# Arcadia-Science/arcadia-microscopy-tools

Measured on AMD Instinct MI355X. Metric: fields-of-view/sec (4x2048^2 uint16) end-to-end segment+props, higher is better.
Workload: dtype f64; 1 GPU; configs[2]: synthetic 4-channel 2048x2048 uint16 FOVs, DAPI Gaussian+Otsu+open/close+EDT+peak markers+watershed nuclei (SEEDED relief, seeds_first: marker pixels spread first in raster order, cannot tie; SURVEY A.8's plain -EDT relief with exact ties is reported under sublines.a8_exact) + clear_border/relabel + morphology and 4-channel intensity regionprops; mode=weak scaling, 192 FOVs per GPU per step, streams_per_gpu=4, fovs_per_launch=48, max_cells_per_fov=2048, distinct_fovs_per_gpu=8, resident_in_hbm=True

## Files before the change

### arcadia_microscopy_tools_amd/csrc/amt_props.hip

```cpp
#include "amt_internal.h"
#include "amt_perlabel.h"

#include <vector>

typedef unsigned long long u64;

enum { A_N = 0, A_SY, A_SX, A_SYY, A_SXX, A_SXY, A_C1, A_C2, A_C3, A_NACC };

__global__ void __launch_bounds__(256) rp_init_kernel(u64* __restrict__ acc, int* __restrict__ bbox, size_t nlab) {
    for (size_t i = (size_t)blockIdx.x * 256 + threadIdx.x; i < nlab; i += (size_t)gridDim.x * 256) {
        if (acc)
            for (int k = 0; k < A_NACC; ++k) acc[i * A_NACC + k] = 0;
        bbox[i * 4 + 0] = 0x7fffffff;
        bbox[i * 4 + 1] = 0x7fffffff;
        bbox[i * 4 + 2] = -1;
        bbox[i * 4 + 3] = -1;
    }
}

__device__ __forceinline__ double diff_of_products(u64 a, u64 b, u64 c, u64 d) {
    u64 lo1 = a * b, hi1 = __umul64hi(a, b);
    u64 lo2 = c * d, hi2 = __umul64hi(c, d);
    bool neg = (hi1 < hi2) || (hi1 == hi2 && lo1 < lo2);
    u64 hi, lo;
    if (!neg) {
        lo = lo1 - lo2;
        hi = hi1 - hi2 - (lo1 < lo2 ? 1 : 0);
    } else {
        lo = lo2 - lo1;
        hi = hi2 - hi1 - (lo2 < lo1 ? 1 : 0);
    }
    double v = (double)hi * 18446744073709551616.0 + (double)lo;
    return neg ? -v : v;
}

__global__ void __launch_bounds__(256) rp_bbox_kernel(const int* __restrict__ labels, int* __restrict__ bbox, int H,
                                                      int W, int max_label) {
    const int lane = threadIdx.x & 63;
    const int x = blockIdx.x * 64 + lane;
    const int yb = (blockIdx.y * 4 + (threadIdx.x >> 6)) * 8;
    if (yb >= H) return;
    const size_t n = (size_t)H * W;
    const int plane = blockIdx.z;
    int labs[8];
#pragma unroll
    for (int k = 0; k < 8; ++k) {
        const int y = yb + k;
        int v = 0;
        if (x < W && y < H) v = labels[(size_t)plane * n + (size_t)y * W + x];
        labs[k] = (v < 0 || v > max_label) ? 0 : v;
    }
#pragma unroll
    for (int k = 0; k < 8; ++k) {
        const int lab = labs[k];
        const int left = __shfl_up(lab, 1);
        const bool head = (lane == 0) || (left != lab);
        const u64 heads = __ballot(head);
        if (lab != 0 && head) {
            const u64 later = heads & ~((2ull << lane) - 1ull);
            const int end_lane = later ? (__ffsll((long long)later) - 2) : 63;
            int* B = bbox + ((size_t)plane * max_label + (lab - 1)) * 4;
            atomicMin(&B[0], yb + k);
            atomicMin(&B[1], x);
            atomicMax(&B[2], yb + k);
            atomicMax(&B[3], x + (end_lane - lane));
        }
    }
}

int amt_i_label_boxes(amt_ctx* ctx, const int* labels, int* bbox, unsigned long long* acc, int nplanes, int H, int W,
                      int max_label) {
    const size_t nlab = (size_t)nplanes * max_label;
    hipLaunchKernelGGL(rp_init_kernel, dim3(amt_grid_for(nlab, 256, 1024)), dim3(256), 0, ctx->stream, acc, bbox, nlab);
    AMT_LAUNCH_CHECK();
    hipLaunchKernelGGL(rp_bbox_kernel, dim3((W + 63) / 64, (H + 31) / 32, nplanes), dim3(256), 0, ctx->stream, labels, bbox,
                       H, W, max_label);
    AMT_LAUNCH_CHECK();
    return AMT_OK;
}

constexpr int RP_MAXC = 4;
constexpr int RPS = 3;
__device__ __forceinline__ size_t rp_uniform(size_t v) {
    const unsigned lo = (unsigned)__builtin_amdgcn_readfirstlane((int)(unsigned)v);
    const unsigned hi = (unsigned)__builtin_amdgcn_readfirstlane((int)(unsigned)(v >> 32));
    return ((size_t)hi << 32) | lo;
}
struct RpSums {
    u64 cnt, sy, sx, syy, sxx, sxy;
    u64 s[RP_MAXC], q[RP_MAXC];
    unsigned mn[RP_MAXC], mx[RP_MAXC];
};

template <int LC>
__device__ __forceinline__ void rp_label_scan(const int* __restrict__ L, const uint16_t* __restrict__ I, size_t n, int W,
                                              int x0, int y0, int x1, int y1, int want, int nc, bool rows_ok,
                                              int2* __restrict__ myrows, int lane, RpSums& a) {
    constexpr int COLS = 1 << LC, RW = 64 >> LC;
    const int col = lane & (COLS - 1), sub = lane >> LC;
    size_t cofs[RP_MAXC];
#pragma unroll
    for (int c = 0; c < RP_MAXC; ++c) cofs[c] = rp_uniform((size_t)(c < nc ? c : 0) * n);
    int lv[RPS];
    unsigned iv[RPS][RP_MAXC] = {};
    auto load_step = [&](int yb, int xb) {
        const int xr = x1 - xb;
        const unsigned cx = (unsigned)(col <= xr ? col : xr);
#pragma unroll
        for (int j = 0; j < RPS; ++j) {
            const int yt = yb + j * RW, ys = yt <= y1 ? yt : y1;
            const int y = yt + sub, yc = y <= y1 ? y : y1;
            const unsigned off = (unsigned)(yc - ys) * (unsigned)W + cx;
            const size_t base = (size_t)ys * W + xb;
            lv[j] = *(const int*)((const char*)(L + base) + off * 4u);
            if (I) {
#pragma unroll
                for (int c = 0; c < RP_MAXC; ++c)
                    iv[j][c] = *(const uint16_t*)((const char*)(I + cofs[c] + base) + off * 2u);
            }
        }
    };
    int nyb = y0, nxb = x0;
    int rmin[RPS], rmax[RPS];
    unsigned tcnt = 0;
    u64 tsy = 0;
    do {
        const int yb = nyb, xb = nxb;
        load_step(yb, xb);
        nxb = xb + 64;
        if (LC < 6 || nxb > x1) {
            nxb = x0;
            nyb = yb + RPS * RW;
        }
        const int x = xb + col;
        if (LC == 6 && xb == x0) {
#pragma unroll
            for (int j = 0; j < RPS; ++j) {
                rmin[j] = 0x7fffffff;
                rmax[j] = -1;
            }
        }
        unsigned bcnt = 0, bsy = 0;
        int2* steprows = myrows + (yb - y0 + sub);
#pragma unroll
        for (int j = 0; j < RPS; ++j) {
            const int y = yb + j * RW + sub;
            const bool m = x <= x1 && y <= y1 && lv[j] == want;
            if (m) {
                bcnt += 1u;
                bsy += (unsigned)y;
                a.syy += (u64)(unsigned)y * (unsigned)y;
                if (I) {
#pragma unroll
                    for (int c = 0; c < RP_MAXC; ++c) {
                        const unsigned v = iv[j][c];
                        a.s[c] += v;
                        a.q[c] += (u64)v * v;
                        a.mn[c] = v < a.mn[c] ? v : a.mn[c];
                        a.mx[c] = v > a.mx[c] ? v : a.mx[c];
                    }
                }
            }
            const u64 bal = __ballot(m);
            if constexpr (LC == 6) {
                if (bal) {
                    const int first = xb + __ffsll((long long)bal) - 1;
                    const int last = xb + 63 - __clzll((long long)bal);
                    rmin[j] = first < rmin[j] ? first : rmin[j];
                    rmax[j] = last > rmax[j] ? last : rmax[j];
                }
            } else {
                const unsigned sm = (unsigned)(bal >> (sub * COLS)) & (0xffffffffu >> (32 - COLS));
                if (rows_ok && col == 0 && y <= y1)
                    steprows[j * RW] = sm ? make_int2(x0 + __ffs((int)sm) - 1, x0 + 31 - __clz((int)sm))
                                          : make_int2(0x7fffffff, -1);
            }
        }
        if constexpr (LC == 6) {
            a.cnt += bcnt;
            a.sy += bsy;
            a.sx += (u64)(unsigned)x * bcnt;
            a.sxx += (u64)(unsigned)x * (unsigned)x * bcnt;
            a.sxy += (u64)(unsigned)x * bsy;
            if (rows_ok && lane == 0 && nxb == x0) {
#pragma unroll
                for (int j = 0; j < RPS; ++j)
                    if (yb + j <= y1) myrows[yb + j - y0] = make_int2(rmin[j], rmax[j]);
            }
        } else {
            tcnt += bcnt;
            tsy += bsy;
        }
    } while (nyb <= y1);
    if constexpr (LC < 6) {
        const unsigned x = (unsigned)(x0 + col);
        a.cnt = tcnt;
        a.sy = tsy;
        a.sx = (u64)x * tcnt;
        a.sxx = (u64)x * x * tcnt;
        a.sxy = (u64)x * tsy;
    }
}

__global__ void __launch_bounds__(64) rp_label_kernel(const int* __restrict__ labels, const int* __restrict__ bbox,
                                                      const int* __restrict__ hoff, const int* __restrict__ htot,
                                                      int2* __restrict__ rows, size_t cap, u64* __restrict__ acc,
                                                      const uint16_t* __restrict__ inten, int C, int c0, int nc,
                                                      double* __restrict__ itable, int H, int W, int max_label,
                                                      int want_morph) {
    const int plane = blockIdx.y;
    const int l = blockIdx.x;
    const int lane = threadIdx.x;
    const size_t li = (size_t)plane * max_label + l;
    const amt_box box = amt_load_box(bbox, li);
    const int y0 = box.y0, x0 = box.x0, y1 = box.y1, x1 = box.x1;
    if (box.absent()) {
        if (itable) amt_fill_row(itable + (li * C + c0) * 4, 4 * nc, 0.0, lane);
        return;
    }
    const size_t n = (size_t)H * W;
    const int* L = labels + (size_t)plane * n;
    const uint16_t* I = inten ? inten + ((size_t)plane * C + c0) * n : nullptr;
    const bool rows_ok = want_morph && (size_t)htot[plane] <= cap;
    int2* myrows = rows + (size_t)plane * cap + (size_t)hoff[li];
    RpSums a;
    a.cnt = a.sy = a.sx = a.syy = a.sxx = a.sxy = 0;
#pragma unroll
    for (int c = 0; c < RP_MAXC; ++c) {
        a.s[c] = 0;
        a.q[c] = 0;
        a.mn[c] = 0xffffffffu;
        a.mx[c] = 0;
    }
    const int w = W < (1 << 28) ? x1 - x0 + 1 : 64;
    if (w <= 16) rp_label_scan<4>(L, I, n, W, x0, y0, x1, y1, l + 1, nc, rows_ok, myrows, lane, a);
    else if (w <= 32) rp_label_scan<5>(L, I, n, W, x0, y0, x1, y1, l + 1, nc, rows_ok, myrows, lane, a);
    else rp_label_scan<6>(L, I, n, W, x0, y0, x1, y1, l + 1, nc, rows_ok, myrows, lane, a);
    static_assert(A_N == 0 && A_SXY == 5, "the moment sums are the first six accumulator slots");
    u64 t[16];
    t[A_N] = a.cnt, t[A_SY] = a.sy, t[A_SX] = a.sx, t[A_SYY] = a.syy, t[A_SXX] = a.sxx, t[A_SXY] = a.sxy;
    unsigned e[2 * RP_MAXC];
#pragma unroll
    for (int c = 0; c < RP_MAXC; ++c) {
        t[6 + c] = a.s[c];
        t[6 + RP_MAXC + c] = a.q[c];
        e[c] = a.mn[c];
        e[RP_MAXC + c] = ~a.mx[c];
    }
    t[14] = t[15] = 0;
    const u64 red = amt_wave_reduce_scatter<16, amt_op_sum>(t, lane);
    if (want_morph && (lane & 3) == 0 && lane < 4 * 6) acc[li * A_NACC + (lane >> 2)] = red;
    if (itable) {
        const unsigned ext = amt_wave_reduce_scatter<8, amt_op_min>(e, lane);
        const u64 cnt = __shfl(red, 0), S = __shfl(red, 4 * (6 + lane)), Q = __shfl(red, 4 * (6 + RP_MAXC + lane));
        const unsigned lo = __shfl(ext, 8 * lane), hi = ~__shfl(ext, 8 * (RP_MAXC + lane));
        if (lane < nc) {
            double* o = itable + (li * C + c0 + lane) * 4;
            if (cnt == 0) {
                o[0] = o[1] = o[2] = o[3] = 0.0;
            } else {
                const double dn = (double)cnt;
                o[0] = (double)S / dn;
                o[1] = (double)hi;
                o[2] = (double)lo;
                const double nv = diff_of_products(cnt, Q, S, S);
                const double var = nv / (dn * dn);
                o[3] = sqrt(var < 0.0 ? 0.0 : var);
            }
        }
    }
}

constexpr int PR_ROWS = 64, PR_IN = 60, PR_BATCH = 17, PR_NBATCH = (PR_ROWS + 4) / PR_BATCH;
static_assert(PR_BATCH * PR_NBATCH == PR_ROWS + 4, "row batches must tile the strip");

__global__ void __launch_bounds__(256) rp_perimeter_rows_kernel(const int* __restrict__ labels, u64* __restrict__ acc,
                                                                int H, int W, int max_label, int* __restrict__ bbox) {
    const int lane = threadIdx.x & 63;
    const int strip = blockIdx.x * 4 + (threadIdx.x >> 6);
    if (strip * PR_IN >= W) return;
    const int plane = blockIdx.z;
    const size_t n = (size_t)H * W;
    const int* L = labels + (size_t)plane * n;
    const int x = strip * PR_IN - 2 + lane;
    const int y0 = blockIdx.y * PR_ROWS;
    const bool xin = x >= 0 && x < W;
    const bool inner = xin && lane >= 2 && lane < 2 + PR_IN;
    const unsigned ml = (unsigned)max_label;
    u64* accp = acc + (size_t)plane * max_label * A_NACC;
    int* bbp = bbox ? bbox + (size_t)plane * max_label * 4 : nullptr;

    const int xc = x < 0 ? 0 : (x < W ? x : W - 1);
    auto load_row = [&](int y) -> int {
        const int yc = y < 0 ? 0 : (y < H ? y : H - 1);
        return L[(size_t)yc * W + xc];
    };
    int cur[PR_BATCH], nxt[PR_BATCH];
#pragma unroll
    for (int j = 0; j < PR_BATCH; ++j) cur[j] = load_row(y0 - 2 + j);
    int v1 = 0, v1l = 0, v1r = 0, v2 = 0, v2l = 0, v2r = 0;
    int wA = 0, wAl = 0, wAr = 0, wB = 0, wBl = 0, wBr = 0;
    for (int b = 0; b < PR_NBATCH; ++b) {
        if (b + 1 < PR_NBATCH) {
#pragma unroll
            for (int j = 0; j < PR_BATCH; ++j) nxt[j] = load_row(y0 - 2 + (b + 1) * PR_BATCH + j);
        }
#pragma unroll
        for (int j = 0; j < PR_BATCH; ++j) {
            const int r = y0 - 2 + b * PR_BATCH + j;
            int v0 = cur[j];
            v0 = (xin && r >= 0 && r < H && (unsigned)(v0 - 1) < ml) ? v0 : 0;
            if (__ballot((v0 | v1 | v2 | wB) != 0) == 0ull) continue;
            const int v0l = amt_lane_left(v0), v0r = amt_lane_right(v0);
            const bool b1 = v1 != 0 && (v2 != v1 || v0 != v1 || v1l != v1 || v1r != v1);
            const int w1 = b1 ? (v1 | (int)0x80000000) : v1;
            const int w1l = amt_lane_left(w1), w1r = amt_lane_right(w1);
            const int yb = r - 1;
            if (bbp && yb >= y0 && yb < y0 + PR_ROWS) {
                const bool live = inner && v1 != 0, head = live && v1l != v1;
                const bool q0 = head && v2 != v1, q2 = head && v0 != v1, q1 = head && v2l != v1 && v0l != v1;
                const bool q3 = live && v1r != v1 && v2r != v1 && v0r != v1;
                if (__ballot(q0 || q1 || q2 || q3)) {
                    int* B = bbp + (size_t)(v1 - 1) * 4;
                    if (q0) atomicMin(&B[0], yb);
                    if (q2) atomicMax(&B[2], yb);
                    if (q1) atomicMin(&B[1], x);
                    if (q3) atomicMax(&B[3], x);
                }
            }
            const int yo = r - 2;
            if (inner && wA < 0 && yo >= y0 && yo < y0 + PR_ROWS) {
                const int key = wA;
                const int code = 1 + 2 * ((wB == key) + (w1 == key) + (wAl == key) + (wAr == key)) +
                                 10 * ((wBl == key) + (wBr == key) + (w1l == key) + (w1r == key));
                constexpr unsigned long long M1 = (1ull << 5) | (1ull << 7) | (1ull << 15) | (1ull << 17) | (1ull << 25) | (1ull << 27);
                constexpr unsigned long long M2 = (1ull << 21) | (1ull << 33), M3 = (1ull << 13) | (1ull << 23);
                const int cls = ((M1 >> code) & 1ull) ? A_C1 : ((M2 >> code) & 1ull) ? A_C2 : ((M3 >> code) & 1ull) ? A_C3 : -1;
                if (cls >= 0) atomicAdd(&accp[(size_t)((key & 0x7fffffff) - 1) * A_NACC + cls], 1ull);
            }
            wB = wA, wBl = wAl, wBr = wAr;
            wA = w1, wAl = w1l, wAr = w1r;
            v2 = v1, v2l = v1l, v2r = v1r;
            v1 = v0, v1l = v0l, v1r = v0r;
        }
#pragma unroll
        for (int j = 0; j < PR_BATCH; ++j) cur[j] = nxt[j];
    }
}

__global__ void __launch_bounds__(256) rp_heights_kernel(const int* __restrict__ bbox, int* __restrict__ hoff,
                                                         int max_label) {
    const int plane = blockIdx.y;
    for (int l = blockIdx.x * 256 + threadIdx.x; l < max_label; l += gridDim.x * 256) {
        const int* B = bbox + ((size_t)plane * max_label + l) * 4;
        hoff[(size_t)plane * max_label + l] = B[2] >= B[0] ? B[2] - B[0] + 1 : 0;
    }
}

constexpr int HULL_HMAX = 48, HULL_WMAX = 250;

__device__ __forceinline__ void rp_write_convex(double* __restrict__ trow, double convex) {
    const double area = trow[AMT_RP_AREA];
    trow[AMT_RP_AREA_CONVEX] = convex;
    trow[AMT_RP_SOLIDITY] = area > 0.0 ? area / convex : 0.0;
}

__device__ __forceinline__ long long floor_div(long long a, long long b) {
    long long q = a / b;
    return (a % b != 0 && a < 0) ? q - 1 : q;
}
__device__ __forceinline__ long long ceil_div(long long a, long long b) {
    long long q = a / b;
    return (a % b != 0 && a > 0) ? q + 1 : q;
}

template <bool CROWS>
__global__ void __launch_bounds__(64) rp_hull_kernel(const int* __restrict__ bbox, const int* __restrict__ hoff,
                                                     const int* __restrict__ htot, const int2* __restrict__ rows,
                                                     int2* __restrict__ chainL, int2* __restrict__ chainR, size_t cap,
                                                     double* __restrict__ table, int max_label, int skip_h,
                                                     int2* __restrict__ crows) {
    const int plane = blockIdx.y;
    const int l = blockIdx.x * 64 + threadIdx.x;
    if (l >= max_label) return;
    const size_t li = (size_t)plane * max_label + l;
    double* trow = CROWS ? nullptr : table + li * AMT_RP_NCOLS;
    const int miny = bbox[li * 4 + 0], maxy = bbox[li * 4 + 2];
    if (maxy < miny) {
        if (!CROWS && skip_h == 0) trow[AMT_RP_AREA_CONVEX] = 0.0;
        return;
    }
    const int h = maxy - miny + 1;
    if (h <= skip_h && bbox[li * 4 + 3] - bbox[li * 4 + 1] + 1 <= HULL_WMAX) return;
    const size_t off = (size_t)hoff[li];
    if ((size_t)htot[plane] > cap || off + (size_t)h > cap) {
        if (!CROWS) rp_write_convex(trow, __longlong_as_double(0x7ff8000000000000ll));
        return;
    }
    const int2* r = rows + (size_t)plane * cap + off;
// ... 209 lines not shown
        const double SQ2 = 1.4142135623730951;
        t[AMT_RP_PERIMETER] = (double)A[A_C1] + (double)A[A_C2] * SQ2 + (double)A[A_C3] * ((1.0 + SQ2) / 2.0);
        const double Nyy = diff_of_products(n, A[A_SYY], A[A_SY], A[A_SY]);
        const double Nxx = diff_of_products(n, A[A_SXX], A[A_SX], A[A_SX]);
        const double Nxy = diff_of_products(n, A[A_SXY], A[A_SX], A[A_SY]);
        const double n2 = dn * dn;
        const double a = Nxx / n2;
        const double c = Nyy / n2;
        const double b = -Nxy / n2;
        const double tr = (a + c) * 0.5;
        const double hd = (a - c) * 0.5;
        const double rad = sqrt(hd * hd + b * b);
        double l1 = tr + rad, l2 = tr - rad;
        l1 = l1 < 0.0 ? 0.0 : l1;
        l2 = l2 < 0.0 ? 0.0 : l2;
        t[AMT_RP_AXIS_MAJOR] = 4.0 * sqrt(l1);
        t[AMT_RP_AXIS_MINOR] = 4.0 * sqrt(l2);
        t[AMT_RP_ECCENTRICITY] = l1 == 0.0 ? 0.0 : sqrt(1.0 - l2 / l1);
        double orient;
        if (Nxx == Nyy) {
            orient = (Nxy > 0.0) ? -0.78539816339744828 : 0.78539816339744828;
        } else {
            orient = 0.5 * atan2(-2.0 * b, c - a);
        }
        t[AMT_RP_ORIENTATION] = orient;
    }
}

extern "C" int amt_regionprops(amt_ctx* ctx, const int32_t* labels, const uint16_t* intensity, int C, double* table_dev,
                               double* itable_dev, int nplanes, int H, int W, int max_label) {
    AMT_REQUIRE(labels && (table_dev || itable_dev) && nplanes >= 0 && H > 0 && W > 0 && max_label >= 0,
                "regionprops: bad arguments");
    AMT_REQUIRE(!intensity == !itable_dev && (!itable_dev || C >= 1),
                "regionprops: the intensity planes (C >= 1) and the intensity table go together");
    AMT_CHECK_OPERANDS("amt_regionprops", amt_in("labels", labels, amt_span(4, nplanes, H, W)),
                       amt_in("intensity", intensity, amt_span(2, nplanes, C, H, W)),
                       amt_out("table_dev", table_dev, amt_span(8, nplanes, max_label, AMT_RP_NCOLS)),
                       amt_out("itable_dev", itable_dev, amt_span(8, nplanes, max_label, C, 4)));
    AMT_TRY(amt_set_device(ctx));
    const bool want_morph = table_dev != nullptr;
    if (nplanes == 0 || max_label == 0) return AMT_OK;
    const size_t n = (size_t)H * W;
    const size_t nlab = (size_t)nplanes * max_label;
    const size_t cap = want_morph ? n : 1;
    amt_scratch s(ctx);
    amt_buf<u64> acc(s, nlab * A_NACC);
    amt_buf<int> bbox(s, nlab * 4);
    amt_buf<int> hoff(s, nlab);
    amt_buf<int> htot(s, nplanes);
    amt_buf<int2> rows(s, (size_t)nplanes * cap);
    amt_buf<int2> chainL(s, (size_t)nplanes * 3 * cap);
    amt_buf<int2> chainR(s, (size_t)nplanes * 3 * cap);
    AMT_TRY(s.commit());
    if (want_morph) {
        hipLaunchKernelGGL(rp_init_kernel, dim3(amt_grid_for(nlab, 256, 1024)), dim3(256), 0, ctx->stream, acc, bbox, nlab);
        AMT_LAUNCH_CHECK();
        const int nstrips = (W + PR_IN - 1) / PR_IN;
        dim3 gper((nstrips + 3) / 4, (H + PR_ROWS - 1) / PR_ROWS, nplanes);
        hipLaunchKernelGGL(rp_perimeter_rows_kernel, gper, dim3(256), 0, ctx->stream, labels, acc, H, W, max_label, bbox);
        AMT_LAUNCH_CHECK();
    } else {
        AMT_TRY(amt_i_label_boxes(ctx, labels, bbox, acc, nplanes, H, W, max_label));
    }
    hipLaunchKernelGGL(rp_heights_kernel, dim3(amt_grid_for(max_label, 256, 256), nplanes), dim3(256), 0, ctx->stream,
                       bbox, hoff, max_label);
    AMT_LAUNCH_CHECK();
    AMT_TRY(amt_scan_excl(ctx, hoff, max_label, (size_t)max_label, htot, nplanes));
    const int groups = intensity ? (C + RP_MAXC - 1) / RP_MAXC : 1;
    for (int g = 0; g < groups; ++g) {
        const int c0 = g * RP_MAXC;
        const int nc = intensity ? ((C - c0) < RP_MAXC ? (C - c0) : RP_MAXC) : 0;
        hipLaunchKernelGGL(rp_label_kernel, dim3(max_label, nplanes), dim3(64), 0, ctx->stream, labels, bbox, hoff, htot,
                           rows, cap, acc, intensity, C, c0, nc, intensity ? itable_dev : (double*)nullptr, H, W,
                           max_label, (want_morph && g == 0) ? 1 : 0);
        AMT_LAUNCH_CHECK();
    }
    if (want_morph) {
        hipLaunchKernelGGL(rp_final_kernel, dim3(amt_grid_for(nlab, 256, 1024)), dim3(256), 0, ctx->stream, acc, bbox,
                           table_dev, nlab);
        AMT_LAUNCH_CHECK();
        const int skip_h = HULL_HMAX;
        hipLaunchKernelGGL(rp_hull_lds_kernel<false>, dim3((max_label + 31) / 32, nplanes), dim3(64), 0, ctx->stream, bbox,
                           hoff, htot, rows, cap, table_dev, max_label, (int2*)nullptr);
        AMT_LAUNCH_CHECK();
        hipLaunchKernelGGL(rp_hull_kernel<false>, dim3((max_label + 63) / 64, nplanes), dim3(64), 0, ctx->stream, bbox,
                           hoff, htot, rows, chainL, chainR, cap, table_dev, max_label, skip_h, (int2*)nullptr);
        AMT_LAUNCH_CHECK();
    }
    return AMT_OK;
}

__global__ void __launch_bounds__(64) rp_intensity_f64_kernel(const int* __restrict__ labels, const int* __restrict__ bbox,
                                                              const double* __restrict__ inten, int C,
                                                              double* __restrict__ itable, int H, int W, int max_label) {
    const int plane = blockIdx.y, l = blockIdx.x, lane = threadIdx.x;
    const size_t li = (size_t)plane * max_label + l;
    const amt_box box = amt_load_box(bbox, li);
    const int y0 = box.y0, x0 = box.x0, y1 = box.y1, x1 = box.x1;
    double* out = itable + li * (size_t)C * 4;
    if (box.absent()) {
        amt_fill_row(out, C * 4, 0.0, lane);
        return;
    }
    const size_t n = (size_t)H * W;
    const int* lab = labels + (size_t)plane * n;
    for (int c = 0; c < C; ++c) {
        const double* img = inten + ((size_t)plane * C + c) * n;
        double s = 0.0, cnt = 0.0, mn = __longlong_as_double(0x7ff0000000000000ll), mx = -mn;
        for (int y = y0; y <= y1; ++y)
            for (int x = x0 + lane; x <= x1; x += 64)
                if (lab[(size_t)y * W + x] == l + 1) {
                    const double v = img[(size_t)y * W + x];
                    s += v;
                    cnt += 1.0;
                    mn = v < mn ? v : mn;
                    mx = v > mx ? v : mx;
                }
        s = amt_wave_sum(s);
        cnt = amt_wave_sum(cnt);
        mn = amt_wave_min(mn);
        mx = amt_wave_max(mx);
        const double mean = s / cnt;
        double q = 0.0;
        for (int y = y0; y <= y1; ++y)
            for (int x = x0 + lane; x <= x1; x += 64)
                if (lab[(size_t)y * W + x] == l + 1) {
                    const double d = img[(size_t)y * W + x] - mean;
// ... 814 lines not shown
```

Before: 16240 FOV/s.

## Rewrite perimeter kernel as bit-packed 64-row column masks with popcount classification

The perimeter/bbox kernel now sweeps 64 rows per lane and packs neighbor-equality predicates into 64-bit column masks. Border and perimeter classes are then derived with bitwise adder logic, and atomics are issued only for the set bits, with labels reloaded at those rows. Tiles overlap by 4 rows (60 useful rows each), and the 1D grid is remapped across the 8 XCDs to improve L2 locality. This replaces per-row shuffle and compare work with word-level logic, at the cost of redundant halo loads and extra label reloads at output rows.

```diff
diff --git a/arcadia_microscopy_tools_amd/csrc/amt_perimeter_bits.h b/arcadia_microscopy_tools_amd/csrc/amt_perimeter_bits.h
--- /dev/null
+++ b/arcadia_microscopy_tools_amd/csrc/amt_perimeter_bits.h
@@ -0,0 +1,48 @@
+#pragma once
+#include <stdint.h>
+
+#if defined(__HIPCC__)
+#define AMT_PB_FN __host__ __device__ __forceinline__
+#else
+#define AMT_PB_FN inline
+#endif
+
+#define AMT_PB_ROWS 0x3ffffffffffffffcull
+
+AMT_PB_FN uint64_t amt_pb_border(uint64_t M, uint64_t Eh, uint64_t EhL, uint64_t Ev) {
+    return M & ~(Eh & EhL & Ev & (Ev >> 1));
+}
+
+AMT_PB_FN void amt_pb_add4(uint64_t a, uint64_t b, uint64_t c, uint64_t d, uint64_t& s0, uint64_t& s1, uint64_t& s2) {
+    const uint64_t x = a ^ b, y = c ^ d, p = a & b, q = c & d, t = x & y;
+    s0 = x ^ y;
+    s1 = p ^ q ^ t;
+    s2 = p & q;
+}
+
+struct amt_pb_out {
+    uint64_t c1, c2, c3;
+    uint64_t q0, q1, q2, q3;
+};
+
+AMT_PB_FN amt_pb_out amt_pb_classify(uint64_t M, uint64_t B, uint64_t BL, uint64_t BR, uint64_t Eh, uint64_t EhL,
+                                     uint64_t Ev, uint64_t Ed1, uint64_t Ed1R, uint64_t Ed2, uint64_t Ed2L,
+                                     uint64_t rows) {
+    const uint64_t up = Ev, dn = Ev >> 1, lf = EhL, rt = Eh;
+    const uint64_t ul = Ed1, ur = Ed2, lr = Ed1R >> 1, ll = Ed2L >> 1;
+    uint64_t a0, a1, a2, d0, d1, d2;
+    amt_pb_add4(up & (B << 1), dn & (B >> 1), lf & BL, rt & BR, a0, a1, a2);
+    amt_pb_add4(ul & (BL << 1), ur & (BR << 1), lr & (BR >> 1), ll & (BL >> 1), d0, d1, d2);
+    const uint64_t out = B & rows;
+    const uint64_t c4_is1 = a0 & ~a1;
+    amt_pb_out o;
+    o.c1 = out & a1 & ~d2 & ~(d1 & d0);
+    o.c2 = out & ((~(a0 | a1 | a2) & d1 & ~d0) | (c4_is1 & d1 & d0));
+    o.c3 = out & c4_is1 & (d0 ^ d1);
+    const uint64_t live = M & rows, head = live & ~lf;
+    o.q0 = head & ~up;
+    o.q2 = head & ~dn;
+    o.q1 = head & ~ul & ~ll;
+    o.q3 = live & ~rt & ~ur & ~lr;
+    return o;
+}
diff --git a/arcadia_microscopy_tools_amd/csrc/amt_props.hip b/arcadia_microscopy_tools_amd/csrc/amt_props.hip
--- a/arcadia_microscopy_tools_amd/csrc/amt_props.hip
+++ b/arcadia_microscopy_tools_amd/csrc/amt_props.hip
@@ -1,6 +1,8 @@
 #include "amt_internal.h"
+#include "amt_perimeter_bits.h"
 #include "amt_perlabel.h"
 
+#include <type_traits>
 #include <vector>
 
 typedef unsigned long long u64;
@@ -271,80 +273,122 @@
     }
 }
 
-constexpr int PR_ROWS = 64, PR_IN = 60, PR_BATCH = 17, PR_NBATCH = (PR_ROWS + 4) / PR_BATCH;
-static_assert(PR_BATCH * PR_NBATCH == PR_ROWS + 4, "row batches must tile the strip");
+constexpr int PR_ROWS = 64, PR_IN = 60, PR_BATCH = 16, PR_NBATCH = PR_ROWS / PR_BATCH, PR_POP = 4;
+constexpr unsigned PR_XCDS = 8;
+static_assert(PR_BATCH * PR_NBATCH == PR_ROWS && PR_IN + 4 == PR_ROWS, "row batches must tile the 64 rows of a word");
+
+__device__ __forceinline__ int pr_lane_left(int v) { return __builtin_amdgcn_update_dpp(0, v, 0x138, 0xf, 0xf, true); }
+__device__ __forceinline__ int pr_lane_right(int v) { return __builtin_amdgcn_update_dpp(0, v, 0x130, 0xf, 0xf, true); }
+
+__device__ __forceinline__ void pr_nonzero5(const int (&x)[5], unsigned (&d)[5]) {
+    asm("v_min_u32_e32 %0, 1, %5\n\tv_min_u32_e32 %1, 1, %6\n\tv_min_u32_e32 %2, 1, %7\n\tv_min_u32_e32 %3, 1, %8\n\t"
+        "v_min_u32_e32 %4, 1, %9"
+        : "=&v"(d[0]), "=&v"(d[1]), "=&v"(d[2]), "=&v"(d[3]), "=&v"(d[4])
+        : "v"(x[0]), "v"(x[1]), "v"(x[2]), "v"(x[3]), "v"(x[4]));
+}
 
 __global__ void __launch_bounds__(256) rp_perimeter_rows_kernel(const int* __restrict__ labels, u64* __restrict__ acc,
-                                                                int H, int W, int max_label, int* __restrict__ bbox) {
+                                                                int H, int W, int max_label, int* __restrict__ bbox,
+                                                                unsigned nplanes) {
     const int lane = threadIdx.x & 63;
-    const int strip = blockIdx.x * 4 + (threadIdx.x >> 6);
+    const unsigned chunk = gridDim.x / PR_XCDS, g = (blockIdx.x % PR_XCDS) * chunk + blockIdx.x / PR_XCDS;
+    const unsigned gx = ((unsigned)(W + PR_IN - 1) / PR_IN + 3) / 4, gy = (unsigned)(H + PR_IN - 1) / PR_IN;
+    const unsigned plane = g / (gx * gy), gyx = g % (gx * gy), ty = gyx / gx;
+    if (plane >= nplanes) return;
+    const int strip = (int)(gyx % gx) * 4 + (threadIdx.x >> 6);
     if (strip * PR_IN >= W) return;
-    const int plane = blockIdx.z;
     const size_t n = (size_t)H * W;
     const int* L = labels + (size_t)plane * n;
     const int x = strip * PR_IN - 2 + lane;
-    const int y0 = blockIdx.y * PR_ROWS;
+    const int y0 = (int)ty * PR_IN - 2;
     const bool xin = x >= 0 && x < W;
     const bool inner = xin && lane >= 2 && lane < 2 + PR_IN;
-    const unsigned ml = (unsigned)max_label;
+    unsigned ml = xin ? (unsigned)max_label : 0u;
+    asm volatile("" : "+v"(ml));
     u64* accp = acc + (size_t)plane * max_label * A_NACC;
     int* bbp = bbox ? bbox + (size_t)plane * max_label * 4 : nullptr;
 
+    unsigned m[2] = {0u, 0u}, nh[2] = {0u, 0u}, nv[2] = {0u, 0u}, n1r[2] = {0u, 0u}, n2l[2] = {0u, 0u};
     const int xc = x < 0 ? 0 : (x < W ? x : W - 1);
-    auto load_row = [&](int y) -> int {
-        const int yc = y < 0 ? 0 : (y < H ? y : H - 1);
-        return L[(size_t)yc * W + xc];
+    auto sweep = [&](auto reaches_out) {
+        constexpr bool EDGE = decltype(reaches_out)::value;
+        const int* rowp = L + (size_t)(y0 < 0 ? 0 : y0) * W;
+        int yl = y0;
+        auto load_row = [&]() -> int {
+            const int v = rowp[xc];
+            if (!EDGE || (yl >= 0 && yl + 1 < H)) rowp += W;
+            ++yl;
+            return v;
+        };
+        int cur[PR_BATCH], nxt[PR_BATCH];
+#pragma unroll
+        for (int j = 0; j < PR_BATCH; ++j) cur[j] = load_row();
+        int above = 0;
+#pragma unroll
+        for (int b = 0; b < PR_NBATCH; ++b) {
+            if (b + 1 < PR_NBATCH) {
+#pragma unroll
+                for (int j = 0; j < PR_BATCH; ++j) nxt[j] = load_row();
+            }
+#pragma unroll
+            for (int j = 0; j < PR_BATCH; ++j) {
+                const int r = b * PR_BATCH + j, h = r >> 5, sh = r & 31;
+                int v0 = cur[j];
+                v0 = (unsigned)(v0 - 1) < ml ? v0 : 0;
+                const int p = above;
+                above = v0;
+                if (__ballot((v0 | p) != 0) == 0ull) continue;
+                const int v0l = pr_lane_left(v0), v0r = pr_lane_right(v0);
+                const int x5[5] = {v0, v0 ^ v0r, v0 ^ p, v0r ^ p, v0l ^ p};
+                unsigned d5[5];
+                pr_nonzero5(x5, d5);
+                m[h] |= d5[0] << sh, nh[h] |= d5[1] << sh, nv[h] |= d5[2] << sh, n1r[h] |= d5[3] << sh, n2l[h] |= d5[4] << sh;
+            }
+#pragma unroll
+            for (int j = 0; j < PR_BATCH; ++j) cur[j] = nxt[j];
+        }
     };
-    int cur[PR_BATCH], nxt[PR_BATCH];
-#pragma unroll
-    for (int j = 0; j < PR_BATCH; ++j) cur[j] = load_row(y0 - 2 + j);
-    int v1 = 0, v1l = 0, v1r = 0, v2 = 0, v2l = 0, v2r = 0;
-    int wA = 0, wAl = 0, wAr = 0, wB = 0, wBl = 0, wBr = 0;
-    for (int b = 0; b < PR_NBATCH; ++b) {
-        if (b + 1 < PR_NBATCH) {
-#pragma unroll
-            for (int j = 0; j < PR_BATCH; ++j) nxt[j] = load_row(y0 - 2 + (b + 1) * PR_BATCH + j);
-        }
-#pragma unroll
-        for (int j = 0; j < PR_BATCH; ++j) {
-            const int r = y0 - 2 + b * PR_BATCH + j;
-            int v0 = cur[j];
-            v0 = (xin && r >= 0 && r < H && (unsigned)(v0 - 1) < ml) ? v0 : 0;
-            if (__ballot((v0 | v1 | v2 | wB) != 0) == 0ull) continue;
-            const int v0l = amt_lane_left(v0), v0r = amt_lane_right(v0);
-            const bool b1 = v1 != 0 && (v2 != v1 || v0 != v1 || v1l != v1 || v1r != v1);
-            const int w1 = b1 ? (v1 | (int)0x80000000) : v1;
-            const int w1l = amt_lane_left(w1), w1r = amt_lane_right(w1);
-            const int yb = r - 1;
-            if (bbp && yb >= y0 && yb < y0 + PR_ROWS) {
-                const bool live = inner && v1 != 0, head = live && v1l != v1;
-                const bool q0 = head && v2 != v1, q2 = head && v0 != v1, q1 = head && v2l != v1 && v0l != v1;
-                const bool q3 = live && v1r != v1 && v2r != v1 && v0r != v1;
-                if (__ballot(q0 || q1 || q2 || q3)) {
-                    int* B = bbp + (size_t)(v1 - 1) * 4;
-                    if (q0) atomicMin(&B[0], yb);
-                    if (q2) atomicMax(&B[2], yb);
-                    if (q1) atomicMin(&B[1], x);
-                    if (q3) atomicMax(&B[3], x);
-                }
-            }
-            const int yo = r - 2;
-            if (inner && wA < 0 && yo >= y0 && yo < y0 + PR_ROWS) {
-                const int key = wA;
-                const int code = 1 + 2 * ((wB == key) + (w1 == key) + (wAl == key) + (wAr == key)) +
-                                 10 * ((wBl == key) + (wBr == key) + (w1l == key) + (w1r == key));
-                constexpr unsigned long long M1 = (1ull << 5) | (1ull << 7) | (1ull << 15) | (1ull << 17) | (1ull << 25) | (1ull << 27);
-                constexpr unsigned long long M2 = (1ull << 21) | (1ull << 33), M3 = (1ull << 13) | (1ull << 23);
-                const int cls = ((M1 >> code) & 1ull) ? A_C1 : ((M2 >> code) & 1ull) ? A_C2 : ((M3 >> code) & 1ull) ? A_C3 : -1;
-                if (cls >= 0) atomicAdd(&accp[(size_t)((key & 0x7fffffff) - 1) * A_NACC + cls], 1ull);
-            }
-            wB = wA, wBl = wAl, wBr = wAr;
-            wA = w1, wAl = w1l, wAr = w1r;
-            v2 = v1, v2l = v1l, v2r = v1r;
-            v1 = v0, v1l = v0l, v1r = v0r;
-        }
-#pragma unroll
-        for (int j = 0; j < PR_BATCH; ++j) cur[j] = nxt[j];
+    if (y0 >= 0 && y0 + PR_ROWS <= H) sweep(std::false_type{});
+    else sweep(std::true_type{});
+    const int rlo = y0 < 0 ? -y0 : 0, rhi = H - y0 < PR_ROWS ? H - y0 : PR_ROWS;
+    const u64 rows = (rhi < 64 ? (1ull << rhi) - 1 : ~0ull) & (~0ull << rlo), pairs = rows & (rows << 1);
+    auto word = [](const unsigned (&w)[2]) { return ((u64)w[1] << 32) | w[0]; };
+    const long long M = (long long)(word(m) & rows), Eh = (long long)~word(nh), Ev = (long long)(~word(nv) & pairs);
+    const long long Ed1R = (long long)(~word(n1r) & pairs), Ed2L = (long long)(~word(n2l) & pairs);
+    if (__ballot(M != 0) == 0ull) return;
+    const long long EhL = amt_lane_left(Eh);
+    const long long B = (long long)amt_pb_border((u64)M, (u64)Eh, (u64)EhL, (u64)Ev);
+    const amt_pb_out o = amt_pb_classify((u64)M, (u64)B, (u64)amt_lane_left(B), (u64)amt_lane_right(B), (u64)Eh, (u64)EhL,
+                                         (u64)Ev, (u64)amt_lane_left(Ed1R), (u64)Ed1R, (u64)amt_lane_right(Ed2L), (u64)Ed2L,
+                                         inner ? AMT_PB_ROWS : 0ull);
+    static_assert(A_C1 + 2 == A_C3 && A_C2 + 1 == A_C3, "the class slots are consecutive");
+    const u64 cls = o.c1 | o.c2 | o.c3, box = bbp ? (o.q0 | o.q1 | o.q2 | o.q3) : 0ull;
+    u64 todo = cls | box;
+    while (todo != 0ull) {
+        int r[PR_POP], lab[PR_POP];
+        bool has[PR_POP];
+#pragma unroll
+        for (int k = 0; k < PR_POP; ++k) {
+            has[k] = todo != 0ull;
+            r[k] = has[k] ? __builtin_ctzll(todo) : r[0];
+            todo &= todo - 1;
+            lab[k] = L[(size_t)(y0 + r[k]) * W + x];
+        }
+#pragma unroll
+        for (int k = 0; k < PR_POP; ++k) {
+            const int y = y0 + r[k];
+            if (has[k] && ((cls >> r[k]) & 1ull)) {
+                const int slot = A_C3 - (int)((o.c2 >> r[k]) & 1ull) - 2 * (int)((o.c1 >> r[k]) & 1ull);
+                atomicAdd(&accp[(size_t)(lab[k] - 1) * A_NACC + slot], 1ull);
+            }
+            if (has[k] && ((box >> r[k]) & 1ull)) {
+                int* Bx = bbp + (size_t)(lab[k] - 1) * 4;
+                if ((o.q0 >> r[k]) & 1ull) atomicMin(&Bx[0], y);
+                if ((o.q2 >> r[k]) & 1ull) atomicMax(&Bx[2], y);
+                if ((o.q1 >> r[k]) & 1ull) atomicMin(&Bx[1], x);
+                if ((o.q3 >> r[k]) & 1ull) atomicMax(&Bx[3], x);
+            }
+        }
     }
 }
 
@@ -663,9 +707,11 @@
     if (want_morph) {
         hipLaunchKernelGGL(rp_init_kernel, dim3(amt_grid_for(nlab, 256, 1024)), dim3(256), 0, ctx->stream, acc, bbox, nlab);
         AMT_LAUNCH_CHECK();
-        const int nstrips = (W + PR_IN - 1) / PR_IN;
-        dim3 gper((nstrips + 3) / 4, (H + PR_ROWS - 1) / PR_ROWS, nplanes);
-        hipLaunchKernelGGL(rp_perimeter_rows_kernel, gper, dim3(256), 0, ctx->stream, labels, acc, H, W, max_label, bbox);
+        const size_t ngroups = (size_t)(((W + PR_IN - 1) / PR_IN + 3) / 4) * ((H + PR_IN - 1) / PR_IN) * nplanes;
+        const size_t nblocks = (ngroups + PR_XCDS - 1) / PR_XCDS * PR_XCDS;
+        AMT_REQUIRE(nblocks <= 0x7fffffffull, "regionprops: too many tiles for one launch");
+        hipLaunchKernelGGL(rp_perimeter_rows_kernel, dim3((unsigned)nblocks), dim3(256), 0, ctx->stream, labels, acc, H, W,
+                           max_label, bbox, (unsigned)nplanes);
         AMT_LAUNCH_CHECK();
     } else {
         AMT_TRY(amt_i_label_boxes(ctx, labels, bbox, acc, nplanes, H, W, max_label));
```

Result: no change. 16360 FOV/s (median of 6 runs) (+0.7%).

## Fold perimeter class counting into per-label scan and vectorize bbox kernel

Applied to the files above, without the earlier changes.

Drops the separate full-image perimeter-rows kernel, which used global 64-bit atomics per border pixel. Perimeter classes are now computed inside the per-label scan from ballot bitmasks kept in an LDS ring buffer, using bitwise neighbour counting, then reduced across the wave. The bounding-box kernel is rewritten to read four labels per lane with int4 loads over taller strips and to issue atomics only at extreme pixels. Banding adds __syncthreads and extra LDS traffic to the per-label kernel. Very wide labels fall back to a slow plain per-pixel path.

```diff
diff --git a/arcadia_microscopy_tools_amd/csrc/amt_props.hip b/arcadia_microscopy_tools_amd/csrc/amt_props.hip
--- a/arcadia_microscopy_tools_amd/csrc/amt_props.hip
+++ b/arcadia_microscopy_tools_amd/csrc/amt_props.hip
@@ -34,37 +34,93 @@
     return neg ? -v : v;
 }
 
-__global__ void __launch_bounds__(256) rp_bbox_kernel(const int* __restrict__ labels, int* __restrict__ bbox, int H,
-                                                      int W, int max_label) {
+constexpr int BX_ROWS = 30, BX_COLS = 256, BX_BATCH = 4, BX_NBATCH = (BX_ROWS + 2) / BX_BATCH;
+static_assert(BX_BATCH * BX_NBATCH == BX_ROWS + 2, "row batches must tile the strip");
+
+template <bool VEC>
+__global__ void __launch_bounds__(256) rp_boxes_kernel(const int* __restrict__ labels, int* __restrict__ bbox, int H,
+                                                       int W, int max_label) {
     const int lane = threadIdx.x & 63;
-    const int x = blockIdx.x * 64 + lane;
-    const int yb = (blockIdx.y * 4 + (threadIdx.x >> 6)) * 8;
-    if (yb >= H) return;
-    const size_t n = (size_t)H * W;
+    const int strip = blockIdx.x * 4 + (threadIdx.x >> 6);
+    if (strip > (W - 1) / BX_COLS) return;
     const int plane = blockIdx.z;
-    int labs[8];
-#pragma unroll
-    for (int k = 0; k < 8; ++k) {
-        const int y = yb + k;
-        int v = 0;
-        if (x < W && y < H) v = labels[(size_t)plane * n + (size_t)y * W + x];
-        labs[k] = (v < 0 || v > max_label) ? 0 : v;
-    }
-#pragma unroll
-    for (int k = 0; k < 8; ++k) {
-        const int lab = labs[k];
-        const int left = __shfl_up(lab, 1);
-        const bool head = (lane == 0) || (left != lab);
-        const u64 heads = __ballot(head);
-        if (lab != 0 && head) {
-            const u64 later = heads & ~((2ull << lane) - 1ull);
-            const int end_lane = later ? (__ffsll((long long)later) - 2) : 63;
-            int* B = bbox + ((size_t)plane * max_label + (lab - 1)) * 4;
-            atomicMin(&B[0], yb + k);
-            atomicMin(&B[1], x);
-            atomicMax(&B[2], yb + k);
-            atomicMax(&B[3], x + (end_lane - lane));
-        }
+    const int* L = labels + (size_t)plane * H * W;
+    int* bbp = bbox + (size_t)plane * max_label * 4;
+    const unsigned x = (unsigned)strip * BX_COLS + 4u * lane;
+    const unsigned uw = (unsigned)W, ml = (unsigned)max_label;
+    const int ya = blockIdx.y * BX_ROWS, yend = ya + BX_ROWS < H ? ya + BX_ROWS : H;
+
+    unsigned xc[4], mlx[4];
+#pragma unroll
+    for (int k = 0; k < 4; ++k) {
+        xc[k] = x + k < uw ? x + k : uw - 1u;
+        mlx[k] = x + k < uw ? ml : 0u;
+    }
+    const unsigned xv = x < uw ? x : uw - 4u;
+    auto load_row = [&](int y) -> int4 {
+        const int yc = y < 0 ? 0 : (y < H ? y : H - 1);
+        const int* row = L + (size_t)yc * W;
+        if constexpr (VEC) return *(const int4*)(row + xv);
+        else return make_int4(row[xc[0]], row[xc[1]], row[xc[2]], row[xc[3]]);
+    };
+    int4 cur[BX_BATCH], nxt[BX_BATCH];
+#pragma unroll
+    for (int j = 0; j < BX_BATCH; ++j) cur[j] = load_row(ya - 1 + j);
+    int c[6] = {}, u[6] = {};
+    for (int b = 0; b < BX_NBATCH; ++b) {
+        if (ya - 1 + b * BX_BATCH > yend) break;
+        if (b + 1 < BX_NBATCH) {
+#pragma unroll
+            for (int j = 0; j < BX_BATCH; ++j) nxt[j] = load_row(ya - 1 + (b + 1) * BX_BATCH + j);
+        }
+#pragma unroll
+        for (int j = 0; j < BX_BATCH; ++j) {
+            const int r = ya - 1 + b * BX_BATCH + j;
+            const bool rin = r >= 0 && r < H;
+            const int raw[4] = {cur[j].x, cur[j].y, cur[j].z, cur[j].w};
+            int d[6];
+#pragma unroll
+            for (int k = 0; k < 4; ++k) {
+                const unsigned top = rin ? mlx[VEC ? 0 : k] : 0u;
+                d[k + 1] = (unsigned)raw[k] <= top ? raw[k] : 0;
+            }
+            d[0] = amt_lane_left(d[4]);
+            d[5] = amt_lane_right(d[1]);
+            const int yc = r - 1;
+            if (yc >= ya && yc < yend && __ballot((c[1] | c[2] | c[3] | c[4]) != 0) != 0ull) {
+                unsigned q0[4], q1[4], q2[4], q3[4], qk[4], any = 0u;
+#pragma unroll
+                for (int k = 1; k <= 4; ++k) {
+                    const unsigned v = (unsigned)c[k];
+                    const unsigned cl = c[k - 1] ^ v, cr = c[k + 1] ^ v, uu = u[k] ^ v, dd = d[k] ^ v;
+                    const unsigned ul = u[k - 1] ^ v, dl = d[k - 1] ^ v, ur = u[k + 1] ^ v, dr = d[k + 1] ^ v;
+                    q0[k - 1] = min(min(v, cl), uu);
+                    q2[k - 1] = min(min(v, cl), dd);
+                    q1[k - 1] = min(min(min(cl, ul), dl), v);
+                    q3[k - 1] = min(min(min(cr, ur), dr), v);
+                    qk[k - 1] = q0[k - 1] | q1[k - 1] | q2[k - 1] | q3[k - 1];
+                    any |= qk[k - 1];
+                }
+                if (__ballot(any != 0u)) {
+#pragma unroll
+                    for (int k = 0; k < 4; ++k) {
+                        if (!qk[k]) continue;
+                        int* B = bbp + (size_t)(c[k + 1] - 1) * 4;
+                        if (q0[k]) atomicMin(&B[0], yc);
+                        if (q2[k]) atomicMax(&B[2], yc);
+                        if (q1[k]) atomicMin(&B[1], (int)(x + k));
+                        if (q3[k]) atomicMax(&B[3], (int)(x + k));
+                    }
+                }
+            }
+#pragma unroll
+            for (int k = 0; k < 6; ++k) {
+                u[k] = c[k];
+                c[k] = d[k];
+            }
+        }
+#pragma unroll
+        for (int j = 0; j < BX_BATCH; ++j) cur[j] = nxt[j];
     }
 }
 
@@ -73,14 +129,20 @@
     const size_t nlab = (size_t)nplanes * max_label;
     hipLaunchKernelGGL(rp_init_kernel, dim3(amt_grid_for(nlab, 256, 1024)), dim3(256), 0, ctx->stream, acc, bbox, nlab);
     AMT_LAUNCH_CHECK();
-    hipLaunchKernelGGL(rp_bbox_kernel, dim3((W + 63) / 64, (H + 31) / 32, nplanes), dim3(256), 0, ctx->stream, labels, bbox,
-                       H, W, max_label);
+    const int nstrips = (W - 1) / BX_COLS + 1;
+    const dim3 grid((nstrips + 3) / 4, (H - 1) / BX_ROWS + 1, nplanes);
+    if ((uintptr_t)labels % 16 == 0 && W % 4 == 0)
+        hipLaunchKernelGGL(rp_boxes_kernel<true>, grid, dim3(256), 0, ctx->stream, labels, bbox, H, W, max_label);
+    else
+        hipLaunchKernelGGL(rp_boxes_kernel<false>, grid, dim3(256), 0, ctx->stream, labels, bbox, H, W, max_label);
     AMT_LAUNCH_CHECK();
     return AMT_OK;
 }
 
 constexpr int RP_MAXC = 4;
 constexpr int RPS = 3;
+constexpr int RP_PW = 1024, RP_LBMAX = 7, RP_WIDE = 32 << RP_LBMAX;
+__host__ __device__ constexpr int rp_band_rows(int lb) { return (RP_PW >> lb) - 4; }
 __device__ __forceinline__ size_t rp_uniform(size_t v) {
     const unsigned lo = (unsigned)__builtin_amdgcn_readfirstlane((int)(unsigned)v);
     const unsigned hi = (unsigned)__builtin_amdgcn_readfirstlane((int)(unsigned)(v >> 32));
@@ -94,8 +156,9 @@
 
 template <int LC>
 __device__ __forceinline__ void rp_label_scan(const int* __restrict__ L, const uint16_t* __restrict__ I, size_t n, int W,
-                                              int x0, int y0, int x1, int y1, int want, int nc, bool rows_ok,
-                                              int2* __restrict__ myrows, int lane, RpSums& a) {
+                                              int x0, int y0, int x1, int ya, int y1, int want, int nc, bool rows_ok,
+                                              int2* __restrict__ myrows, unsigned* __restrict__ pw, int lb, int lane,
+                                              RpSums& a, unsigned& tcnt, u64& tsy) {
     constexpr int COLS = 1 << LC, RW = 64 >> LC;
     const int col = lane & (COLS - 1), sub = lane >> LC;
     size_t cofs[RP_MAXC];
@@ -120,10 +183,8 @@
             }
         }
     };
-    int nyb = y0, nxb = x0;
+    int nyb = ya, nxb = x0;
     int rmin[RPS], rmax[RPS];
-    unsigned tcnt = 0;
-    u64 tsy = 0;
     do {
         const int yb = nyb, xb = nxb;
         load_step(yb, xb);
@@ -163,6 +224,8 @@
             }
             const u64 bal = __ballot(m);
             if constexpr (LC == 6) {
+                if (pw && lane == 0 && y <= y1)
+                    *(u64*)(pw + (((y - y0) & ((RP_PW - 1) >> lb)) << lb) + ((xb - x0) >> 5)) = bal;
                 if (bal) {
                     const int first = xb + __ffsll((long long)bal) - 1;
                     const int last = xb + 63 - __clzll((long long)bal);
@@ -174,6 +237,7 @@
                 if (rows_ok && col == 0 && y <= y1)
                     steprows[j * RW] = sm ? make_int2(x0 + __ffs((int)sm) - 1, x0 + 31 - __clz((int)sm))
                                           : make_int2(0x7fffffff, -1);
+                if (pw && col == 0 && y <= y1) pw[(y - y0) & (RP_PW - 1)] = sm;
             }
         }
         if constexpr (LC == 6) {
@@ -192,8 +256,103 @@
             tsy += bsy;
         }
     } while (nyb <= y1);
+}
+
+__device__ __forceinline__ void rp_sum4(unsigned p, unsigned q, unsigned r, unsigned t, unsigned& s0, unsigned& s1,
+                                        unsigned& s2) {
+    const unsigned x1 = p ^ q, c1 = p & q, x2 = r ^ t, c2 = r & t, k = x1 & x2;
+    s0 = x1 ^ x2;
+    s1 = c1 ^ c2 ^ k;
+    s2 = c1 & c2;
+}
+template <bool MULTI>
+__device__ __forceinline__ void rp_perimeter_rows(const unsigned* __restrict__ pw, int lb, int nw, int y0, int ylast,
+                                                  int ya, int yb, int lane, unsigned (&cls)[3]) {
+    const int rmask = (RP_PW - 1) >> lb;
+    for (int i = lane; i < (yb - ya + 1) << lb; i += 64) {
+        const int y = ya + (i >> lb), b = MULTI ? i & ((1 << lb) - 1) : 0;
+        if (MULTI && b >= nw) continue;
+        unsigned m[5];
+        unsigned lf[5], rt[5];
+#pragma unroll
+        for (int r = 0; r < 5; ++r) {
+            const int yy = y - 2 + r;
+            const bool ok = yy >= y0 && yy <= ylast;
+            const int base = (((yy - y0) & rmask) << lb) + b;
+            const unsigned mc = pw[base];
+            m[r] = ok ? mc : 0u;
+            lf[r] = rt[r] = 0u;
+            if constexpr (MULTI) {
+                const unsigned ml = pw[base - (b > 0 ? 1 : 0)], mr = pw[base + (b + 1 < nw ? 1 : 0)];
+                lf[r] = (ok && b > 0) ? ml >> 30 : 0u;
+                rt[r] = (ok && b + 1 < nw) ? mr & 3u : 0u;
+            }
+        }
+        unsigned B[3], wst[3], est[3];
+#pragma unroll
+        for (int r = 0; r < 3; ++r) {
+            const unsigned c = m[r + 1];
+            const unsigned cin_w = lf[r + 1] >> 1, cin_e = (rt[r + 1] & 1u) << 31;
+            B[r] = c & ~(m[r] & m[r + 2] & ((c << 1) | cin_w) & ((c >> 1) | cin_e));
+            const unsigned bl = (lf[r + 1] >> 1) & ~((lf[r] >> 1) & (lf[r + 2] >> 1) & lf[r + 1] & c) & 1u;
+            const unsigned br = rt[r + 1] & ~(rt[r] & rt[r + 2] & (c >> 31) & (rt[r + 1] >> 1)) & 1u;
+            wst[r] = (B[r] << 1) | bl;
+            est[r] = (B[r] >> 1) | (br << 31);
+        }
+        unsigned a0, a1, a2, d0, d1, d2;
+        rp_sum4(B[0], B[2], wst[1], est[1], a0, a1, a2);
+        rp_sum4(wst[0], est[0], wst[2], est[2], d0, d1, d2);
+        const unsigned ctr = B[1];
+        const unsigned a_is1 = a0 & ~a1 & ~a2, d_is2 = d1 & ~d0 & ~d2;
+        cls[0] += (unsigned)__popc(ctr & a1 & ~a2 & ~d2 & ~(d1 & d0));
+        cls[1] += (unsigned)__popc(ctr & ((~(a0 | a1 | a2) & d_is2) | (a_is1 & d1 & d0)));
+        cls[2] += (unsigned)__popc(ctr & a_is1 & ((d0 & ~d1 & ~d2) | d_is2));
+    }
+}
+
+__device__ __forceinline__ void rp_perimeter_plain(const int* __restrict__ L, int H, int W, int x0, int y0, int x1, int y1,
+                                                   int want, int lane, unsigned (&cls)[3]) {
+    auto on = [&](int y, int x) {
+        return (unsigned)y < (unsigned)H && (unsigned)x < (unsigned)W && L[(size_t)y * W + x] == want;
+    };
+    auto border = [&](int y, int x) {
+        return on(y, x) && !(on(y - 1, x) && on(y + 1, x) && on(y, x - 1) && on(y, x + 1));
+    };
+    for (int y = y0; y <= y1; ++y)
+        for (int xb = x0; xb <= x1; xb += 64) {
+            const int x = xb + lane;
+            if (x > x1 || !border(y, x)) continue;
+            const int a = border(y - 1, x) + border(y + 1, x) + border(y, x - 1) + border(y, x + 1);
+            const int d = border(y - 1, x - 1) + border(y - 1, x + 1) + border(y + 1, x - 1) + border(y + 1, x + 1);
+            cls[0] += (a == 2 || a == 3) && d <= 2;
+            cls[1] += (a == 0 && d == 2) || (a == 1 && d == 3);
+            cls[2] += a == 1 && (d == 1 || d == 2);
+        }
+}
+
+template <int LC>
+__device__ __forceinline__ void rp_label_bands(const int* __restrict__ L, const uint16_t* __restrict__ I, size_t n, int W,
+                                               int x0, int y0, int x1, int y1, int want, int nc, bool rows_ok,
+                                               int2* __restrict__ myrows, unsigned* __restrict__ pw, int lb, int nw, int lane,
+                                               RpSums& a, unsigned (&cls)[3]) {
+    const int band = rp_band_rows(lb);
+    unsigned tcnt = 0;
+    u64 tsy = 0;
+    int ya = y0, ycount = y0;
+    do {
+        const int yb = (pw && y1 - ya >= band) ? ya + band - 1 : y1;
+        rp_label_scan<LC>(L, I, n, W, x0, y0, x1, ya, yb, want, nc, rows_ok, myrows, pw, lb, lane, a, tcnt, tsy);
+        if (pw) {
+            __syncthreads();
+            const int yc = yb == y1 ? y1 : yb - 2;
+            rp_perimeter_rows<LC == 6>(pw, lb, nw, y0, yb, ycount, yc, lane, cls);
+            ycount = yc + 1;
+            __syncthreads();
+        }
+        ya = yb + 1;
+    } while (ya <= y1);
     if constexpr (LC < 6) {
-        const unsigned x = (unsigned)(x0 + col);
+        const unsigned x = (unsigned)(x0 + (lane & ((1 << LC) - 1)));
         a.cnt = tcnt;
         a.sy = tsy;
         a.sx = (u64)x * tcnt;
@@ -233,9 +392,16 @@
         a.mx[c] = 0;
     }
     const int w = W < (1 << 28) ? x1 - x0 + 1 : 64;
-    if (w <= 16) rp_label_scan<4>(L, I, n, W, x0, y0, x1, y1, l + 1, nc, rows_ok, myrows, lane, a);
-    else if (w <= 32) rp_label_scan<5>(L, I, n, W, x0, y0, x1, y1, l + 1, nc, rows_ok, myrows, lane, a);
-    else rp_label_scan<6>(L, I, n, W, x0, y0, x1, y1, l + 1, nc, rows_ok, myrows, lane, a);
+    __shared__ __attribute__((aligned(8))) unsigned s_pw[RP_PW];
+    const bool per = (want_morph & 2) != 0;
+    const int nw = w <= 32 ? 1 : (((x1 - x0) >> 6) + 1) * 2, lb = 32 - __clz(nw - 1);
+    const bool ring = per && x1 - x0 < RP_WIDE;
+    unsigned cls[3] = {0u, 0u, 0u};
+    unsigned* pw = ring ? s_pw : nullptr;
+    if (w <= 16) rp_label_bands<4>(L, I, n, W, x0, y0, x1, y1, l + 1, nc, rows_ok, myrows, pw, 0, 1, lane, a, cls);
+    else if (w <= 32) rp_label_bands<5>(L, I, n, W, x0, y0, x1, y1, l + 1, nc, rows_ok, myrows, pw, 0, 1, lane, a, cls);
+    else rp_label_bands<6>(L, I, n, W, x0, y0, x1, y1, l + 1, nc, rows_ok, myrows, pw, lb, nw, lane, a, cls);
+    if (per && !ring) rp_perimeter_plain(L, H, W, x0, y0, x1, y1, l + 1, lane, cls);
     static_assert(A_N == 0 && A_SXY == 5, "the moment sums are the first six accumulator slots");
     u64 t[16];
     t[A_N] = a.cnt, t[A_SY] = a.sy, t[A_SX] = a.sx, t[A_SYY] = a.syy, t[A_SXX] = a.sxx, t[A_SXY] = a.sxy;
@@ -250,6 +416,12 @@
     t[14] = t[15] = 0;
     const u64 red = amt_wave_reduce_scatter<16, amt_op_sum>(t, lane);
     if (want_morph && (lane & 3) == 0 && lane < 4 * 6) acc[li * A_NACC + (lane >> 2)] = red;
+    if (per) {
+        static_assert(A_C2 == A_C1 + 1 && A_C3 == A_C1 + 2, "the class counts are three consecutive accumulator slots");
+        u64 pc[8] = {cls[0], cls[1], cls[2], 0, 0, 0, 0, 0};
+        const u64 pr = amt_wave_reduce_scatter<8, amt_op_sum>(pc, lane);
+        if ((lane & 7) == 0 && lane < 8 * 3) acc[li * A_NACC + A_C1 + (lane >> 3)] = pr;
+    }
     if (itable) {
         const unsigned ext = amt_wave_reduce_scatter<8, amt_op_min>(e, lane);
         const u64 cnt = __shfl(red, 0), S = __shfl(red, 4 * (6 + lane)), Q = __shfl(red, 4 * (6 + RP_MAXC + lane));
@@ -268,83 +440,6 @@
                 o[3] = sqrt(var < 0.0 ? 0.0 : var);
             }
         }
-    }
-}
-
-constexpr int PR_ROWS = 64, PR_IN = 60, PR_BATCH = 17, PR_NBATCH = (PR_ROWS + 4) / PR_BATCH;
-static_assert(PR_BATCH * PR_NBATCH == PR_ROWS + 4, "row batches must tile the strip");
-
-__global__ void __launch_bounds__(256) rp_perimeter_rows_kernel(const int* __restrict__ labels, u64* __restrict__ acc,
-                                                                int H, int W, int max_label, int* __restrict__ bbox) {
-    const int lane = threadIdx.x & 63;
-    const int strip = blockIdx.x * 4 + (threadIdx.x >> 6);
-    if (strip * PR_IN >= W) return;
-    const int plane = blockIdx.z;
-    const size_t n = (size_t)H * W;
-    const int* L = labels + (size_t)plane * n;
-    const int x = strip * PR_IN - 2 + lane;
-    const int y0 = blockIdx.y * PR_ROWS;
-    const bool xin = x >= 0 && x < W;
-    const bool inner = xin && lane >= 2 && lane < 2 + PR_IN;
-    const unsigned ml = (unsigned)max_label;
-    u64* accp = acc + (size_t)plane * max_label * A_NACC;
-    int* bbp = bbox ? bbox + (size_t)plane * max_label * 4 : nullptr;
-
-    const int xc = x < 0 ? 0 : (x < W ? x : W - 1);
-    auto load_row = [&](int y) -> int {
-        const int yc = y < 0 ? 0 : (y < H ? y : H - 1);
-        return L[(size_t)yc * W + xc];
-    };
-    int cur[PR_BATCH], nxt[PR_BATCH];
-#pragma unroll
-    for (int j = 0; j < PR_BATCH; ++j) cur[j] = load_row(y0 - 2 + j);
-    int v1 = 0, v1l = 0, v1r = 0, v2 = 0, v2l = 0, v2r = 0;
-    int wA = 0, wAl = 0, wAr = 0, wB = 0, wBl = 0, wBr = 0;
-    for (int b = 0; b < PR_NBATCH; ++b) {
-        if (b + 1 < PR_NBATCH) {
-#pragma unroll
-            for (int j = 0; j < PR_BATCH; ++j) nxt[j] = load_row(y0 - 2 + (b + 1) * PR_BATCH + j);
-        }
-#pragma unroll
-        for (int j = 0; j < PR_BATCH; ++j) {
-            const int r = y0 - 2 + b * PR_BATCH + j;
-            int v0 = cur[j];
-            v0 = (xin && r >= 0 && r < H && (unsigned)(v0 - 1) < ml) ? v0 : 0;
-            if (__ballot((v0 | v1 | v2 | wB) != 0) == 0ull) continue;
-            const int v0l = amt_lane_left(v0), v0r = amt_lane_right(v0);
-            const bool b1 = v1 != 0 && (v2 != v1 || v0 != v1 || v1l != v1 || v1r != v1);
-            const int w1 = b1 ? (v1 | (int)0x80000000) : v1;
-            const int w1l = amt_lane_left(w1), w1r = amt_lane_right(w1);
-            const int yb = r - 1;
-            if (bbp && yb >= y0 && yb < y0 + PR_ROWS) {
-                const bool live = inner && v1 != 0, head = live && v1l != v1;
-                const bool q0 = head && v2 != v1, q2 = head && v0 != v1, q1 = head && v2l != v1 && v0l != v1;
-                const bool q3 = live && v1r != v1 && v2r != v1 && v0r != v1;
-                if (__ballot(q0 || q1 || q2 || q3)) {
-                    int* B = bbp + (size_t)(v1 - 1) * 4;
-                    if (q0) atomicMin(&B[0], yb);
-                    if (q2) atomicMax(&B[2], yb);
-                    if (q1) atomicMin(&B[1], x);
-                    if (q3) atomicMax(&B[3], x);
-                }
-            }
-            const int yo = r - 2;
-            if (inner && wA < 0 && yo >= y0 && yo < y0 + PR_ROWS) {
-                const int key = wA;
-                const int code = 1 + 2 * ((wB == key) + (w1 == key) + (wAl == key) + (wAr == key)) +
-                                 10 * ((wBl == key) + (wBr == key) + (w1l == key) + (w1r == key));
-                constexpr unsigned long long M1 = (1ull << 5) | (1ull << 7) | (1ull << 15) | (1ull << 17) | (1ull << 25) | (1ull << 27);
-                constexpr unsigned long long M2 = (1ull << 21) | (1ull << 33), M3 = (1ull << 13) | (1ull << 23);
-                const int cls = ((M1 >> code) & 1ull) ? A_C1 : ((M2 >> code) & 1ull) ? A_C2 : ((M3 >> code) & 1ull) ? A_C3 : -1;
-                if (cls >= 0) atomicAdd(&accp[(size_t)((key & 0x7fffffff) - 1) * A_NACC + cls], 1ull);
-            }
-            wB = wA, wBl = wAl, wBr = wAr;
-            wA = w1, wAl = w1l, wAr = w1r;
-            v2 = v1, v2l = v1l, v2r = v1r;
-            v1 = v0, v1l = v0l, v1r = v0r;
-        }
-#pragma unroll
-        for (int j = 0; j < PR_BATCH; ++j) cur[j] = nxt[j];
     }
 }
 
@@ -660,16 +755,7 @@
     amt_buf<int2> chainL(s, (size_t)nplanes * 3 * cap);
     amt_buf<int2> chainR(s, (size_t)nplanes * 3 * cap);
     AMT_TRY(s.commit());
-    if (want_morph) {
-        hipLaunchKernelGGL(rp_init_kernel, dim3(amt_grid_for(nlab, 256, 1024)), dim3(256), 0, ctx->stream, acc, bbox, nlab);
-        AMT_LAUNCH_CHECK();
-        const int nstrips = (W + PR_IN - 1) / PR_IN;
-        dim3 gper((nstrips + 3) / 4, (H + PR_ROWS - 1) / PR_ROWS, nplanes);
-        hipLaunchKernelGGL(rp_perimeter_rows_kernel, gper, dim3(256), 0, ctx->stream, labels, acc, H, W, max_label, bbox);
-        AMT_LAUNCH_CHECK();
-    } else {
-        AMT_TRY(amt_i_label_boxes(ctx, labels, bbox, acc, nplanes, H, W, max_label));
-    }
+    AMT_TRY(amt_i_label_boxes(ctx, labels, bbox, acc, nplanes, H, W, max_label));
     hipLaunchKernelGGL(rp_heights_kernel, dim3(amt_grid_for(max_label, 256, 256), nplanes), dim3(256), 0, ctx->stream,
                        bbox, hoff, max_label);
     AMT_LAUNCH_CHECK();
@@ -680,7 +766,7 @@
         const int nc = intensity ? ((C - c0) < RP_MAXC ? (C - c0) : RP_MAXC) : 0;
         hipLaunchKernelGGL(rp_label_kernel, dim3(max_label, nplanes), dim3(64), 0, ctx->stream, labels, bbox, hoff, htot,
                            rows, cap, acc, intensity, C, c0, nc, intensity ? itable_dev : (double*)nullptr, H, W,
-                           max_label, (want_morph && g == 0) ? 1 : 0);
+                           max_label, (want_morph && g == 0) ? 3 : 0);
         AMT_LAUNCH_CHECK();
     }
     if (want_morph) {
```

Result: faster. 16270 FOV/s before, 16650 FOV/s after, median of 6 (+2.3%).
